# Quantumzhao/ParallelParsing

Hardware: AMD Instinct MI355X
Metric: FASTQ records/sec + decompressed MB/s, 50 GB .fastq.gz, 1/2/4/8 MI355X (higher is better)
Workload: dtype u8

## Files before the change

### parallelparsing_amd/csrc/ppg_inflate.hip

```cpp
#include <hip/hip_runtime.h>
#include <stdint.h>
#include <stdlib.h>
#include <stdio.h>
#include <type_traits>
#include "ppg_device.h"
#include "ppg_huffman.h"
#include <atomic>
#include <mutex>
#define PPG_SORT_SLOT 320

#define IX_RING_BYTES 65536u
#define IX_RING_MASK (IX_RING_BYTES - 1u)

template <int RB, int LBT, typename RingT = uint8_t>
struct __attribute__((aligned(16))) InflateLds {
    uint32_t stream[132];
    RingT ring[1u << RB];
    union {
        uint32_t lit[1 << LBT];
        uint32_t cl[1 << CB];
    };
    uint32_t dst[1 << DB];
    uint8_t lens[320];
    uint32_t cen[8];
    uint16_t dsort[32];
};

#ifdef PPG_IX_STATS
__device__ unsigned long long ppg_ixstat[16];
#endif

#ifdef PPG_STAMPS
__device__ unsigned long long ppg_stamp_acc[25];
#define PPG_STAMP(t) const uint64_t t = __builtin_amdgcn_s_memtime()
#else
#define PPG_STAMP(t)
#endif

__device__ __forceinline__ uint32_t rdlane(uint32_t v, uint32_t lane) {
    return (uint32_t)__builtin_amdgcn_readlane((int)v, (int)lane);
}

extern "C" __device__ int llvm_writelane(int, int, int) __asm("llvm.amdgcn.writelane");

__device__ __forceinline__ uint32_t bperm(uint32_t byte_addr, uint32_t v) {
    return (uint32_t)__builtin_amdgcn_ds_bpermute((int)byte_addr, (int)v);
}

struct Reader {
    const uint32_t *base;
    uint32_t nw;
    uint32_t sg;
    uint32_t wi;
    uint64_t bb;
    uint32_t bn;
};

__device__ __forceinline__ void lds_dma_dword(const uint32_t *src, const uint32_t *lds_base) {
    asm volatile("s_nop 0\n\tglobal_load_lds_dword %0, off" ::"v"(src), "{m0}"((uint32_t)(uintptr_t)lds_base)
                 : "memory");
}

__device__ __forceinline__ void st_issue(const Reader &r, uint32_t *stream, uint32_t g, int lane) {
    const uint32_t i = min(g * 32 + (uint32_t)lane, r.nw - 1);
    if (lane < 32) lds_dma_dword(r.base + i, stream + (g & 3) * 32);
    if ((g & 3) == 0 && lane < 4) lds_dma_dword(r.base + i, stream + 128);
}

__device__ __forceinline__ void st_enter(Reader &r, uint32_t *stream, uint32_t g, int lane) {
    if (g == r.sg || g + 1 == r.sg) return;
    if (g != r.sg + 1) {
        st_issue(r, stream, g, lane);
        st_issue(r, stream, g + 1, lane);
    }
    st_issue(r, stream, g + 2, lane);
    r.sg = g;
    asm volatile("s_waitcnt vmcnt(1)" ::: "memory");
}

__device__ __forceinline__ uint32_t rd_word(Reader &r, uint32_t *stream, uint32_t w, int lane) {
    st_enter(r, stream, w >> 5, lane);
    return uni(stream[w & 127]);
}

__device__ __forceinline__ void rd_seek(Reader &r, uint32_t *stream, uint32_t bit, int lane) {
    r.wi = bit >> 5;
    const uint32_t w = rd_word(r, stream, r.wi, lane);
    r.wi++;
    const uint32_t sh = bit & 31;
    r.bb = (uint64_t)(w >> sh);
    r.bn = 32 - sh;
}

__device__ __forceinline__ void rd_refill(Reader &r, uint32_t *stream, int lane) {
    if (r.bn <= 32) {
        const uint32_t w = rd_word(r, stream, r.wi, lane);
        r.wi++;
        r.bb |= (uint64_t)w << r.bn;
        r.bn += 32;
    }
}

__device__ __forceinline__ uint32_t rd_pos(const Reader &r) { return r.wi * 32 - r.bn; }

template <int RB>
__device__ __forceinline__ void flush_range(const uint8_t *ring, uint8_t *out, uint64_t glo, uint64_t ghi, int lane) {
    constexpr uint64_t RM = (1ull << RB) - 1;
    if (ghi <= glo) return;
    const uint64_t a = (glo + 15) & ~15ull, z = ghi & ~15ull;
    if (a >= z) {
        for (uint64_t g0 = glo; g0 < ghi; g0 += 64) {
            const uint64_t g = g0 + lane;
            if (g < ghi) out[g] = ring[g & RM];
        }
        return;
    }
    if (lane < (int)(a - glo)) out[glo + lane] = ring[(glo + lane) & RM];
    if (lane < (int)(ghi - z)) out[z + lane] = ring[(z + lane) & RM];
    for (uint64_t g0 = a; g0 < z; g0 += 1024) {
        const uint64_t g = g0 + (uint64_t)lane * 16;
        if (g < z) {
            uint4 v = *(const uint4 *)(ring + (g & RM));
            *(uint4 *)(out + g) = v;
        }
    }
}

template <int RB>
__device__ __forceinline__ void flush_range_sym(const uint16_t *ring, uint16_t *out, uint64_t glo, uint64_t ghi,
                                                int lane) {
    constexpr uint64_t RM = (1ull << RB) - 1;
    if (ghi <= glo) return;
    const uint64_t a = (glo + 7) & ~7ull, z = ghi & ~7ull;
    if (a >= z) {
        for (uint64_t g0 = glo; g0 < ghi; g0 += 64) {
            const uint64_t g = g0 + lane;
            if (g < ghi) out[g] = ring[g & RM];
        }
        return;
    }
    if (lane < (int)(a - glo)) out[glo + lane] = ring[(glo + lane) & RM];
    if (lane < (int)(ghi - z)) out[z + lane] = ring[(z + lane) & RM];
    for (uint64_t g0 = a; g0 < z; g0 += 512) {
        const uint64_t g = g0 + (uint64_t)lane * 8;
        if (g < z) *(uint4 *)(out + g) = *(const uint4 *)(ring + (g & RM));
    }
}

#define PPG_FILL 0x41414141u

__device__ __forceinline__ uint32_t zero_bytes(uint32_t x) {
    return ~(((x & 0x7F7F7F7Fu) + 0x7F7F7F7Fu) | x) & 0x80808080u;
}

__device__ __forceinline__ uint32_t nl_mask16(uint32_t w0, uint32_t w1, uint32_t w2, uint32_t w3) {
    const uint32_t n0 = zero_bytes(w0 ^ 0x0A0A0A0Au) >> 7, n1 = zero_bytes(w1 ^ 0x0A0A0A0Au) >> 7;
    const uint32_t n2 = zero_bytes(w2 ^ 0x0A0A0A0Au) >> 7, n3 = zero_bytes(w3 ^ 0x0A0A0A0Au) >> 7;
    const uint32_t lo = __builtin_amdgcn_udot4(n1, 0x80402010u, __builtin_amdgcn_udot4(n0, 0x08040201u, 0u, false), false);
    const uint32_t hi = __builtin_amdgcn_udot4(n3, 0x80402010u, __builtin_amdgcn_udot4(n2, 0x08040201u, 0u, false), false);
    return lo | (hi << 8);
}

__device__ __forceinline__ uint32_t wave_incl_scan(uint32_t x) {
    x += (uint32_t)__builtin_amdgcn_update_dpp(0, (int)x, 0x111, 0xF, 0xF, false);
    x += (uint32_t)__builtin_amdgcn_update_dpp(0, (int)x, 0x112, 0xF, 0xF, false);
    x += (uint32_t)__builtin_amdgcn_update_dpp(0, (int)x, 0x114, 0xF, 0xF, false);
    x += (uint32_t)__builtin_amdgcn_update_dpp(0, (int)x, 0x118, 0xF, 0xF, false);
    x += (uint32_t)__builtin_amdgcn_update_dpp(0, (int)x, 0x142, 0xA, 0xF, false);
    x += (uint32_t)__builtin_amdgcn_update_dpp(0, (int)x, 0x143, 0xC, 0xF, false);
    return x;
}

struct CensusOut {
    uint32_t *dst;
    uint32_t cap;
    uint32_t shift;
};

__device__ __forceinline__ void census_step(uint32_t *cen, const CensusOut &co, uint32_t w0, uint32_t w1, uint32_t w2,
                                            uint32_t w3, uint32_t p_lane, uint32_t lastbit, uint32_t nact, int lane) {
    const uint32_t m = nl_mask16(w0, w1, w2, w3);
    const uint32_t z = zero_bytes(w0) | zero_bytes(w1) | zero_bytes(w2) | zero_bytes(w3);
    const uint64_t L = __ballot((m >> lastbit) & 1u);
    const uint64_t F = __ballot(m & 1u);
    const uint64_t B = __ballot((m & (m << 1)) != 0u);
    const uint64_t Z = __ballot(z != 0u);
    uint32_t cnt = uni(cen[0]);
    const uint32_t prevnl = uni(cen[1]);
    uint32_t flags = uni(cen[2]);
    if (B | Z | (F & ((L << 1) | prevnl))) flags |= PPG_PF_SERIAL;
    if (Z) flags |= PPG_PF_NUL;
    const uint32_t c = (uint32_t)__builtin_popcount(m);
    const uint32_t incl = wave_incl_scan(c);
    const uint32_t total = rdlane(incl, 63);
    if (total) {
        uint32_t idx = cnt + incl - c;
        uint32_t mm = m;
        while (__ballot(mm != 0u)) {
            if (mm) {
                const uint32_t b = (uint32_t)__builtin_ctz(mm);
                mm &= mm - 1u;
                if (idx < co.cap) ((__attribute__((address_space(1))) uint32_t *)co.dst)[idx] = co.shift + p_lane + b;
                idx++;
            }
        }
        cnt += total;
        if (cnt > co.cap) flags |= PPG_PF_OVERFLOW;
    }
    if (lane == 0) {
        cen[0] = cnt;
        cen[1] = (uint32_t)(L >> (nact - 1)) & 1u;
        cen[2] = flags;
    }
}

__device__ __forceinline__ CensusOut census_out(const uint32_t *cen) {
    CensusOut co;
    co.cap = uni(cen[3]);
    co.shift = uni(cen[4]);
    co.dst = (uint32_t *)(((uint64_t)uni(cen[6]) << 32) | uni(cen[5]));
    return co;
}

template <int RB>
__device__ __forceinline__ void flush_census(const uint8_t *ring, uint8_t *out, uint64_t out_off, uint32_t lo,
                                             uint32_t hi, int lane, uint32_t *cen) {
    constexpr uint32_t RM = (1u << RB) - 1;
    const CensusOut co = census_out(cen);
    for (uint32_t p = lo; p < hi;) {
        const uint64_t g = out_off + p;
        const uint32_t left = hi - p;
        const uint32_t head = (uint32_t)(-g & 15);
        uint32_t w0 = PPG_FILL, w1 = PPG_FILL, w2 = PPG_FILL, w3 = PPG_FILL, lastbit, nact;
        if (head == 0 && left >= 16) {
            nact = min(left / 16, 64u);
            if ((uint32_t)lane < nact) {
                const uint4 v = *(const uint4 *)(ring + ((uint32_t)(g + 16 * lane) & RM));
                *(uint4 *)(out + g + 16 * lane) = v;
                w0 = v.x; w1 = v.y; w2 = v.z; w3 = v.w;
            }
            lastbit = 15;
            nact *= 16;
        } else {
            nact = min(head ? head : 64u, left);
            if ((uint32_t)lane < nact) {
                const uint8_t c = ring[(uint32_t)(g + lane) & RM];
                out[g + lane] = c;
                w0 = (PPG_FILL & ~255u) | c;
            }
            lastbit = 0;
        }
        census_step(cen, co, w0, w1, w2, w3, p + (lastbit ? 16 : 1) * (uint32_t)lane, lastbit,
                    lastbit ? nact / 16 : nact, lane);
        p += nact;
    }
}

template <bool IX = false, uint32_t IXM = IX_RING_MASK>
__device__ __forceinline__ uint32_t far_byte(const uint8_t *ob, uint32_t oa, const uint8_t *dict, int32_t p) {
    if constexpr (IX) {
        if (p >= 0) return ((const uint16_t *)ob)[(uint32_t)p & IXM];
        return 32768u + (uint32_t)p;
    } else {
        if (p >= 0) {
            const uint32_t q = oa + (uint32_t)p;
            return (*(const uint32_t *)(ob + (q & ~3u)) >> (8 * (q & 3))) & 255u;
        }
        return dict[32768u + (uint32_t)p];
    }
}

__device__ __forceinline__ uint32_t far_load(const uint8_t *base, uint32_t off) {
    uint32_t v;
    asm volatile("global_load_dword %0, %1, %2\n\ts_waitcnt vmcnt(0)" : "=&v"(v) : "v"(off), "s"(base) : "memory");
    return v;
}
__device__ __forceinline__ uint32_t far_load_u8(const uint8_t *base, uint32_t off) {
    uint32_t v;
    asm volatile("global_load_ubyte %0, %1, %2\n\ts_waitcnt vmcnt(0)" : "=&v"(v) : "v"(off), "s"(base) : "memory");
    return v;
}

template <int RB, bool IX, typename RingT, uint32_t IXM = IX_RING_MASK>
__device__ __forceinline__ void copy_match(RingT *ring, const uint8_t *ob, uint32_t oa, const uint8_t *dict,
                                           uint32_t rb0, uint32_t pos, uint32_t dist, uint32_t n, int lane) {
    constexpr uint32_t RM = (1u << RB) - 1;
    constexpr uint32_t REACH = (1u << RB) - 64;
    const uint32_t dst0 = rb0 + pos;
    if (dist + n <= REACH) {
        const uint32_t src0 = dst0 - dist;
        if (dist >= n) {
            for (uint32_t j0 = 0; j0 < n; j0 += 64) {
                const uint32_t j = j0 + lane;
                if (j < n) ring[(dst0 + j) & RM] = ring[(src0 + j) & RM];
            }
        } else {
            for (uint32_t j0 = 0; j0 < n; j0 += 64) {
                const uint32_t j = j0 + lane;
                if (j < n) ring[(dst0 + j) & RM] = ring[(src0 + j % dist) & RM];
            }
        }
    } else {
        for (uint32_t j0 = 0; j0 < n; j0 += 64) {
            const uint32_t j = j0 + lane;
            if (j < n) {
                const uint32_t back = dist - j;
                const int32_t rel = (int32_t)pos - (int32_t)back;
                uint32_t v;
                if (back + n <= REACH) v = ring[(dst0 - back) & RM];
                else v = far_byte<IX, IXM>(ob, oa, dict, rel);
                ring[(dst0 + j) & RM] = (RingT)v;
            }
        }
    }
}

template <int LBT>
__device__ __forceinline__ uint32_t spec_token(const uint32_t *lit, const uint32_t *dst, uint32_t lo, uint32_t hi,
                                               uint32_t lane) {
    const uint32_t e = lit[lo & ((1u << LBT) - 1)];
    const uint32_t e2 = e >> 8;
    const uint32_t xs = e2 - e;
    const uint32_t y = __builtin_amdgcn_alignbit(hi, lo, e2);
    uint32_t tke;
    asm("v_lshl_add_u32 %0, %1, 8, %2" : "=v"(tke) : "v"(__builtin_amdgcn_ubfe(lo, e, xs)), "v"(e2));
    const uint32_t d = dst[y & ((1u << DB) - 1)];
    const uint32_t dm1 = (d >> 16) + __builtin_amdgcn_ubfe(y, d, d >> 10);
    const uint32_t tlen = tke + ((d >> 5) & 31) + (dm1 << 17);
    const uint32_t lm = (uint32_t)((int32_t)(e << 25) >> 31);
    const uint32_t sd = (uint32_t)((int32_t)d >> 31);
    uint32_t t2, tok;
    asm("v_bfi_b32 %0, %1, %2, %3" : "=v"(t2) : "v"(sd), "v"(PPG_SPECIAL_TOKEN), "v"(tlen));
    asm("v_bfi_b32 %0, %1, %2, %3" : "=v"(tok) : "v"(lm), "v"(t2), "v"(e));
    return tok;
}
__device__ __forceinline__ void walk2_asm(uint32_t va, uint32_t vb, uint32_t &vtin, uint32_t &X, uint32_t &t,
                                          uint32_t &half) {
    uint32_t tmp;
    asm volatile(
        "1:\n\t"
        "v_readlane_b32 %[t], %[va], %[X]\n\t"
        "s_lshr_b32 m0, %[X], 8\n\t"
        "s_add_u32 %[X], %[t], %[X]\n\t"
        "s_and_b32 %[tmp], %[X], 0x1c0c0\n\t"
        "v_writelane_b32 %[vtin], %[t], m0\n\t"
        "s_cbranch_scc1 4f\n\t"
        "v_readlane_b32 %[t], %[va], %[X]\n\t"
        "s_lshr_b32 m0, %[X], 8\n\t"
        "s_add_u32 %[X], %[t], %[X]\n\t"
        "s_and_b32 %[tmp], %[X], 0x1c0c0\n\t"
        "v_writelane_b32 %[vtin], %[t], m0\n\t"
        "s_cbranch_scc0 1b\n"
        "4:\n\t"
        "s_mov_b32 %[h], 0\n\t"
        "s_and_b32 %[tmp], %[X], 0x1c080\n\t"
        "s_cbranch_scc1 3f\n\t"
        "s_sub_u32 %[X], %[X], 64\n\t"
        "s_mov_b32 %[h], 64\n"
        "2:\n\t"
        "v_readlane_b32 %[t], %[vb], %[X]\n\t"
        "s_lshr_b32 m0, %[X], 8\n\t"
        "s_add_u32 %[X], %[t], %[X]\n\t"
        "s_and_b32 %[tmp], %[X], 0x1c0c0\n\t"
        "v_writelane_b32 %[vtin], %[t], m0\n\t"
        "s_cbranch_scc1 3f\n\t"
        "v_readlane_b32 %[t], %[vb], %[X]\n\t"
        "s_lshr_b32 m0, %[X], 8\n\t"
        "s_add_u32 %[X], %[t], %[X]\n\t"
        "s_and_b32 %[tmp], %[X], 0x1c0c0\n\t"
        "v_writelane_b32 %[vtin], %[t], m0\n\t"
        "s_cbranch_scc0 2b\n"
        "3:"
        : [vtin] "+v"(vtin), [X] "+s"(X), [t] "=&s"(t), [tmp] "=&s"(tmp), [h] "=&s"(half)
        : [va] "v"(va), [vb] "v"(vb)
        : "m0", "scc");
}
__device__ __forceinline__ uint32_t latch_limit(uint32_t x, uint32_t lim) {
    uint32_t r;
    asm("s_bitcmp1_b32 %1, 7\n\ts_cselect_b32 %0, 0, %2" : "=s"(r) : "s"(uni(x)), "s"(uni(lim)) : "scc");
    return r;
}


template <int RB, int LBT, bool IX, bool CEN, bool IXF = false>
__global__ __launch_bounds__(64) __attribute__((amdgpu_num_sgpr(80), amdgpu_waves_per_eu(8, 8))) void ppg_inflate_kernel(const uint32_t *__restrict__ comp, uint64_t nwords,
                                                         const PpgInflateJob *__restrict__ jobs,
                                                         const uint8_t *__restrict__ dicts, uint8_t *__restrict__ out,
                                                         PpgInflateResult *__restrict__ res, int njobs,
                                                         PpgBlockEnd *__restrict__ blk, uint32_t *__restrict__ nls,
                                                         uint16_t *__restrict__ gsort) {
    constexpr uint32_t RING = 1u << RB;
    constexpr uint32_t RM = RING - 1;
    constexpr uint32_t UNIT = RB >= 13 ? 4096u : RING / 2;
    static_assert(RB >= 10 && RB <= 15, "ring of 1..32 KiB");
    using RingT = typename std::conditional<IX, uint16_t, uint8_t>::type;
    constexpr uint32_t IXM = IXF ? 0xFFFFFFFFu : IX_RING_MASK;
    static_assert(!IXF || IX, "IXF is a pass-1 (IX) form");
    __shared__ InflateLds<RB, LBT, RingT> S;
    const int lane = threadIdx.x;
    const int k = blockIdx.x;
    if (k >= njobs) return;
    uint16_t *const lit_sorted = gsort + (size_t)k * PPG_SORT_SLOT;
    uint16_t *const dst_sorted = S.dsort;
    uint16_t *const lit_tmp = (uint16_t *)S.dst, *const cl_tmp = (uint16_t *)S.dst, *const dst_tmp = (uint16_t *)S.lens;
#ifdef PPG_STAMPS
    const uint64_t tk0 = __builtin_amdgcn_s_memtime();
    uint64_t sx_spec = 0, sx_nspec = 0, sx_flush = 0, sx_nflush = 0, sx_hdr = 0, sx_nhdr = 0, sx_hp = 0, sx_nhp = 0;
#endif
    const PpgInflateJob J = jobs[k];
    const uint64_t out_off = J.out_off;
    const uint32_t len = IX ? 0xFFFFFFFFu : (uint32_t)J.out_len;
    const uint32_t ixcap = IXF ? (uint32_t)J.out_len : 0xF0000000u;
    const uint32_t rb0 = (uint32_t)out_off;
    const uint8_t *dict = dicts + J.dict_off;
    const uint8_t *ob = IX ? out + 2 * out_off : out + (out_off & ~3ull);
    const uint32_t oa = IX ? 0u : (uint32_t)(out_off & 3);

    if constexpr (IX) {
        for (uint32_t w0 = 0; w0 < RING; w0 += 64) {
            const uint32_t w = w0 + lane;
            S.ring[(rb0 - RING + w) & RM] = (uint16_t)(32768u - RING + w);
        }
    } else {
        for (uint32_t w0 = 0; w0 < RING / 4; w0 += 64) {
            const uint32_t w = w0 + lane;
            const uint32_t v = *(const uint32_t *)(dict + 32768 - RING + 4 * w);
            const uint32_t slot = rb0 - RING + 4 * w;
#pragma unroll
            for (int q = 0; q < 4; q++) S.ring[(slot + q) & RM] = (uint8_t)(v >> (8 * q));
        }
    }
    constexpr bool census = CEN && !IX;
    if (census && lane == 0) {
        const uint64_t d = (uint64_t)(uintptr_t)(nls + J.nl_off);
        S.cen[0] = 0;
        S.cen[1] = J.prev_byte == '\n';
        S.cen[2] = 0;
        S.cen[3] = J.nl_cap;
        S.cen[4] = J.raw_shift;
        S.cen[5] = (uint32_t)d;
        S.cen[6] = (uint32_t)(d >> 32);
    }
    __syncthreads();

    const uint64_t w0abs = (J.bit_start >> 5) & ~127ull;
    Reader r;
    r.sg = 0x7FFFFFF0u;
    r.base = comp + w0abs;
    r.nw = (uint32_t)min(nwords > w0abs ? nwords - w0abs : 1ull, 0xFFFFFFFFull);
    const uint32_t bit_limit = (uint32_t)min(J.bit_limit - w0abs * 32, 0xFFFFFFFFull);
    rd_seek(r, S.stream, (uint32_t)(J.bit_start - w0abs * 32), lane);

    const uint64_t lanes_le = lane == 63 ? ~0ull : ((2ull << lane) - 1ull);

    uint32_t pos = 0;
    uint32_t fl_done = 0;
    uint32_t fl_next = UNIT - (uint32_t)(out_off % UNIT);
    int status = ST_OK, flags = 0, last = 0, in_block = 0;
    Canon clit = {0, 0, 0}, cdst = {0, 0, 0};
#ifdef PPG_IX_STATS
    uint64_t ix_unk = 0;
    uint32_t ix_last = 0;
#endif
    auto flush = [&](uint32_t lo, uint32_t hi) {
        if constexpr (IX) {
#ifdef PPG_IX_STATS
            for (uint32_t p0 = lo; p0 < hi; p0 += 64) {
                const uint32_t p = p0 + (uint32_t)lane;
                const uint64_t b = __ballot(p < hi && S.ring[(rb0 + p) & RM] < 0x8000u);
                ix_unk += (uint64_t)__popcll(b);
                if (b) ix_last = p0 + 64u - (uint32_t)__clzll(b);
            }
#endif
            const uint64_t g = out_off + (lo & IXM);
            flush_range_sym<RB>(S.ring, (uint16_t *)out, g, g + (hi - lo), lane);
        } else {
            if constexpr (census) {
                flush_census<RB>(S.ring, out, out_off, lo, hi, lane, S.cen);
            } else {
                flush_range<RB>(S.ring, out, out_off + lo, out_off + hi, lane);
            }
        }
    };
    uint32_t nblk = 0;
#ifdef PPG_STAMPS
    uint64_t sa_dec = 0, sa_walk = 0, sa_rd = 0, sa_far = 0, sa_dep = 0, sa_tail = 0, sa_rounds = 0, sa_farr = 0;
    uint64_t hs_dec = 0, hs_walk = 0, hs_look = 0, hs_fin = 0, hs_words = 0, hs_emit = 0, hs_rounds = 0;
#endif
#ifdef PPG_STATS
    uint32_t st_rounds = 0, st_tokens = 0, st_spec = 0, st_short = 0, st_far = 0, st_dep = 0, st_dbl = 0,
             st_blit = 0, st_beob = 0, st_bmatch = 0;
#endif
    auto block_end = [&](uint32_t e) -> bool {
        if (nblk >= J.blk_cap) { flags |= PPG_FLAG_BLK_FULL; return false; }
        if (lane == 0) blk[J.blk_off + nblk] = PpgBlockEnd{w0abs * 32 + e, pos};
        nblk++;
        return w0abs * 32 + e < J.stop_bit;
    };


    while (pos < len && !last) {
        r.sg = uni(r.sg);
        r.wi = uni(r.wi);
        r.bb = uni64(r.bb);
        r.bn = uni(r.bn);
        pos = uni(pos);
        fl_done = uni(fl_done);
        fl_next = uni(fl_next);
        status = (int)uni((uint32_t)status);
#ifdef PPG_STAMPS
        const uint64_t th0 = __builtin_amdgcn_s_memtime();
#endif
        rd_refill(r, S.stream, lane);
        last = (int)br_take(r, 1);
        const uint32_t type = br_take(r, 2);
        if (type == 0) {
            br_take(r, r.bn & 7);
            rd_refill(r, S.stream, lane);
            const uint32_t slen = br_take(r, 16), nlen = br_take(r, 16);
            if ((slen ^ 0xFFFFu) != nlen) { status = ST_DATA_ERROR; break; }
            const uint32_t bytepos = rd_pos(r) >> 3;
            const uint8_t *c8 = (const uint8_t *)r.base + bytepos;
            const uint32_t remain = min(slen, len - pos);
            if ((uint64_t)bytepos + remain > (uint64_t)r.nw * 4) { status = ST_DATA_ERROR; break; }
            uint32_t copied = 0;
            while (copied < remain) {
                const uint32_t piece = min(remain - copied, (uint32_t)UNIT);
                for (uint32_t j0 = 0; j0 < piece; j0 += 64) {
                    const uint32_t j = j0 + lane;
                    if (j < piece) S.ring[(rb0 + pos + j) & RM] = (RingT)((IX ? 0x8000u : 0u) | c8[copied + j]);
                }
                pos += piece;
                copied += piece;
                if (pos >= fl_next) {
                    flush(fl_done, fl_next);
                    fl_done = fl_next;
                    fl_next += UNIT;
                }
            }
            rd_seek(r, S.stream, (bytepos + copied) * 8, lane);
            if (copied < slen) break;
            in_block = 0;
            if constexpr (IX) {
                if (!block_end((bytepos + copied) * 8)) break;
            }
            continue;
        }
        if (type == 3) { status = ST_DATA_ERROR; break; }
        if (type == 1) {
            for (int s0 = 0; s0 < 320; s0 += 64) {
                const int s = s0 + lane;
                uint8_t L;
                if (s < 144) L = 8; else if (s < 256) L = 9; else if (s < 280) L = 7; else if (s < 288) L = 8;
                else L = 5;
                S.lens[s] = L;
            }
            __syncthreads();
            build_table<LBT>(S.lens, 288, S.lit, &clit, lit_tmp, TAB_LIT, lane, lit_sorted);
            build_table<DB>(S.lens + 288, 32, S.dst, &cdst, dst_tmp, TAB_DST, lane, dst_sorted);
        } else {
            asm volatile("s_setprio 2");
            rd_refill(r, S.stream, lane);
            const uint32_t hlit = br_take(r, 5) + 257, hdist = br_take(r, 5) + 1, hclen = br_take(r, 4) + 4;
            if (hlit > 286 || hdist > 30) { status = ST_DATA_ERROR; break; }
            if (lane < 19) S.lens[lane] = 0;
            __syncthreads();
            for (uint32_t i = 0; i < hclen; i++) {
                rd_refill(r, S.stream, lane);
                const uint32_t v = br_take(r, 3);
                if (lane == 0) S.lens[c_clorder[i]] = (uint8_t)v;
            }
            __syncthreads();
            if (build_table<CB>(S.lens, 19, S.cl, nullptr, cl_tmp, TAB_CL, lane) != 0) { status = ST_DATA_ERROR; break; }
            uint32_t idx = 0;
            const uint32_t total = hlit + hdist;
            bool bad = false;
            while (idx < total) {
                rd_refill(r, S.stream, lane);
                const uint32_t e = uni(S.cl[(uint32_t)r.bb & ((1u << CB) - 1)]);
                const uint32_t L = e & 15;
                if (L == 0) { bad = true; break; }
                br_take(r, L);
                const uint32_t sym = e >> 8;
                uint32_t val = 0, rep = 1;
                if (sym < 16) { val = sym; }
                else if (sym == 16) {
                    if (idx == 0) { bad = true; break; }
                    val = uni(S.lens[idx - 1]);
                    rep = 3 + br_take(r, 2);
                } else if (sym == 17) { rep = 3 + br_take(r, 3); }
                else { rep = 11 + br_take(r, 7); }
                if (idx + rep > total) { bad = true; break; }
                for (uint32_t j0 = 0; j0 < rep; j0 += 64)
                    if (j0 + lane < rep) S.lens[idx + j0 + lane] = (uint8_t)val;
                idx += rep;
            }
            __syncthreads();
            if (bad) { status = ST_DATA_ERROR; break; }
            if (uni(S.lens[256]) == 0) { status = ST_DATA_ERROR; break; }
            if (build_table<LBT>(S.lens, (int)hlit, S.lit, &clit, lit_tmp, TAB_LIT, lane, lit_sorted) != 0) { status = ST_DATA_ERROR; break; }
            if (build_table<DB>(S.lens + hlit, (int)hdist, S.dst, &cdst, dst_tmp, TAB_DST, lane, dst_sorted) != 0) { status = ST_DATA_ERROR; break; }
        }
        in_block = 1;
#ifdef PPG_STAMPS
        sx_hdr += __builtin_amdgcn_s_memtime() + 0 * (uint64_t)__builtin_amdgcn_readfirstlane(S.lit[lane]) - th0;
        sx_nhdr++;
#endif
        asm volatile("s_setprio 0");
        r.sg = uni(r.sg);
        r.wi = uni(r.wi);
        r.bb = uni64(r.bb);
        r.bn = uni(r.bn);
        pos = uni(pos);
        fl_done = uni(fl_done);
        fl_next = uni(fl_next);

        uint32_t bp = rd_pos(r);
#ifdef PPG_STAMPS
        uint64_t st_w0 = 0;
#endif
        uint32_t cn = 0, cw = 0;

        struct Round { uint32_t vtin, off, adv, tl, xr; };
        struct Words { uint32_t x0, x1, x2, x3, x4; };
        auto words = [&](uint32_t bp) -> Words {
            const uint32_t *sw = S.stream + __builtin_amdgcn_ubfe(bp + (uint32_t)lane, 5u, 7u);
            return Words{sw[0], sw[1], sw[2], sw[3], sw[4]};
        };
        auto decode = [&](auto hot, uint32_t bp, uint32_t cn, uint32_t cw, uint32_t pos, const Words &W) -> Round {
            constexpr bool HOT = decltype(hot)::value;
            uint32_t s = 0, off = cn, t = 0, half = 0;
            uint32_t tl = cw, xr = 0;
            uint32_t vtin = (uint32_t)llvm_writelane((int)cw, 0, 0);
            if (__builtin_expect(off < (HOT ? 64u : min(64u, len - pos)), 1)) {
                const uint32_t o = bp + (uint32_t)lane;
                const uint32_t x0 = W.x0, x1 = W.x1, x2 = W.x2, x3 = W.x3, x4 = W.x4;
                const uint32_t vta = spec_token<LBT>(S.lit, S.dst, __builtin_amdgcn_alignbit(x1, x0, o),
                                                     __builtin_amdgcn_alignbit(x2, x1, o), (uint32_t)lane);
                const uint32_t vtb = spec_token<LBT>(S.lit, S.dst, __builtin_amdgcn_alignbit(x3, x2, o),
                                                     __builtin_amdgcn_alignbit(x4, x3, o), (uint32_t)lane);

                constexpr uint32_t STOP = 0x1C0C0u;
                uint32_t X;
#ifdef PPG_STAMPS
                st_w0 = __builtin_amdgcn_s_memtime() + 0 * (uint64_t)__builtin_amdgcn_readfirstlane(vta ^ vtb);
#endif
                if (HOT || len - pos >= 64) {
                    X = off << 8;
                    asm volatile("s_setprio 2");
                    walk2_asm(vta, vtb, vtin, X, tl, half);
                    if constexpr (!HOT) asm volatile("s_setprio 1");
                    off = (X >> 8) & 511u;
                } else {
                    const uint32_t cl = 64u - (len - pos);
                    X = (off + cl) << 8;
                    do {
                        t = rdlane(vta, X);
                        vtin = (uint32_t)llvm_writelane((int)t, (int)((X >> 8) - cl), (int)vtin);
                        X += t;
                    } while ((X & STOP) == 0u);
                    if ((X & (STOP & ~0x40u)) == 0u) {
                        X -= 64;
                        half = 64;
                        do {
                            t = rdlane(vtb, X);
                            vtin = (uint32_t)llvm_writelane((int)t, (int)((X >> 8) - cl), (int)vtin);
                            X += t;
                        } while ((X & STOP) == 0u);
                    }
                    off = ((X >> 8) & 511u) - cl;
                    tl = t;
                }
                xr = X;
                s = half + (X & 127u);
            }
            return Round{vtin, off, s, tl, xr};
        };

        st_enter(r, S.stream, bp >> 10, lane);
        Words W = words(bp);
        auto one_round = [&]() -> uint32_t {
            constexpr bool HOT = false;
            PPG_STAMP(t0);
            const Round R = decode(std::false_type{}, bp, cn, cw, pos, W);
            st_enter(r, S.stream, (bp + R.adv) >> 10, lane);
            W = words(bp + R.adv);
#ifdef PPG_STAMPS
            const uint64_t t1 = __builtin_amdgcn_s_memtime() + 0 * (uint64_t)__builtin_amdgcn_readfirstlane(R.vtin);
            if (st_w0 < t0) st_w0 = t1;
            sa_dec += st_w0 - t0;
            sa_walk += t1 - st_w0;
            sa_rounds++;
#endif
#ifdef PPG_STATS
            st_rounds++;
            st_tokens += (uint32_t)__popcll(__ballot(R.vtin != 0));
            if (R.xr & 128u) st_spec++;
            if (R.off < 64) st_short++;
#endif
            const uint32_t tot = HOT ? R.off : min(R.off, len - pos);
            const uint32_t rout = min(tot, 64u);
            const uint64_t mo = __ballot(R.vtin != 0);
            {
                uint32_t sj4;
                asm("v_mad_i32_i24 %0, %1, -4, %2" : "=v"(sj4) : "v"((uint32_t)__builtin_clzll(mo & lanes_le)), "s"(252u));
                const uint32_t inf = bperm(sj4, R.vtin);
                const int32_t jj = lane - 1 - (int32_t)(inf >> 17);
                const uint32_t rv = S.ring[(rb0 + pos + (uint32_t)jj) & RM];
                uint32_t val;
                if constexpr (IX) val = ((inf >> 8) & 511u) != 1u ? rv : (0x8000u | ((inf >> 17) & 255u));
                else val = ((inf >> 8) & 511u) != 1u ? rv : ((inf >> 17) & 255u);
                const bool far = jj < -(int32_t)(RING - 64);
                const uint64_t fm = __ballot(far);
#ifdef PPG_STATS
                if (fm) st_far++;
#endif
#ifdef PPG_STAMPS
                const uint64_t t2 = __builtin_amdgcn_s_memtime() + 0 * (uint64_t)__builtin_amdgcn_readfirstlane(val);
                sa_rd += t2 - t1;
#endif
                if (fm) {
                  {
                    const int32_t p = (int32_t)pos + jj;
                    const bool fo = far && p >= 0;
                    if constexpr (IX) {
                        const uint32_t q = 2u * ((uint32_t)p & IXM);
                        const uint32_t w = far_load(ob, fo ? (q & ~3u) : 0u);
                        val = fo ? __builtin_amdgcn_ubfe(w, q << 3, 16u) : val;
                    } else {
                        const uint32_t b = far_load_u8(ob, fo ? (uint32_t)jj + (pos + oa) : 0u);
                        val = fo ? b : val;
                    }
                    const bool fd = far && p < 0;
                    const uint64_t dm = fm & __ballot(p < 0);
                    if (dm) {
                        uint32_t db;
                        if constexpr (IX) db = 32768u + (uint32_t)p;
                        else db = dict[fd ? 32768u + (uint32_t)p : 0u];
                        val = fd ? db : val;
                    }
                  }
                }
#ifdef PPG_STAMPS
                const uint64_t t3 = __builtin_amdgcn_s_memtime() + 0 * (uint64_t)__builtin_amdgcn_readfirstlane(val);
                sa_far += t3 - t2;
                sa_farr += fm ? 1 : 0;
#endif
                const bool dep = jj >= 0;
                if (__ballot(dep)) {
                    int32_t ptr = dep ? jj : lane;
#ifdef PPG_STATS
                    st_dep++;
#endif
                    for (;;) {
#ifdef PPG_STATS
                        st_dbl++;
#endif
                        const int32_t p2 = (int32_t)bperm((uint32_t)ptr << 2, (uint32_t)ptr);
                        if (!__ballot(p2 != ptr)) break;
                        ptr = p2;
                    }
                    val = bperm((uint32_t)ptr << 2, val);
                }
                S.ring[(rb0 + pos + lane) & RM] = (RingT)val;
#ifdef PPG_STAMPS
                const uint64_t t4 = __builtin_amdgcn_s_memtime() + 0 * (uint64_t)__builtin_amdgcn_readfirstlane(val);
                sa_dep += t4 - t3;
                st_w0 = t4;
#endif
            }
            cn = tot - rout;
            cw = R.tl & ~(511u << 8);
            pos += rout;
            bp += R.adv;
            asm volatile("s_setprio 0");
            if constexpr (IX) {
                if (bp > bit_limit || pos > ixcap) { status = ST_DATA_ERROR; return 128u; }
            }
#ifdef PPG_STAMPS
            sa_tail += __builtin_amdgcn_s_memtime() + 0 * (uint64_t)bp - st_w0;
            st_w0 = 0;
#endif
            return R.xr;
        };
        auto hot_pipe = [&](auto early, uint32_t limh) -> uint32_t {
            constexpr bool EARLY = decltype(early)::value;
            uint32_t p_val = 0, p_b = 0, p_pos = pos, lim_r;
            int32_t p_jj = -1;
            auto finish = [&]() {
                uint32_t val = p_val;
                if constexpr (IX) {
                    const uint32_t q = 2u * ((p_pos + (uint32_t)p_jj) & IXM);
                    uint32_t fv = __builtin_amdgcn_ubfe(p_b, q << 3, 16u);
                    if constexpr (EARLY) {
                        const int32_t p = (int32_t)p_pos + p_jj;
                        fv = p < 0 ? 32768u + (uint32_t)p : fv;
                    }
                    val = p_jj < -(int32_t)(RING - 64) ? fv : val;
                } else {
                    val = p_jj < -(int32_t)(RING - 64) ? p_b : val;
                }
                const bool dep = p_jj >= 0;
                if (__ballot(dep)) {
                    int32_t ptr = dep ? p_jj : lane;
                    for (;;) {
                        const int32_t p2 = (int32_t)bperm((uint32_t)ptr << 2, (uint32_t)ptr);
                        if (!__ballot(p2 != ptr)) break;
                        ptr = p2;
                    }
                    val = bperm((uint32_t)ptr << 2, val);
                }
                S.ring[(rb0 + p_pos + lane) & RM] = (RingT)val;
            };
            do {
                PPG_STAMP(h0);
                const Round R = decode(std::true_type{}, bp, cn, cw, pos, W);
#ifdef PPG_STAMPS
                const uint64_t h1 = __builtin_amdgcn_s_memtime() + 0 * (uint64_t)__builtin_amdgcn_readfirstlane(R.vtin);
                if (st_w0 < h0) st_w0 = h1;
                hs_dec += st_w0 - h0;
                hs_walk += h1 - st_w0;
                hs_rounds++;
#endif
                const uint32_t rout = min(R.off, 64u);
                const uint64_t mo = __ballot(R.vtin != 0);
                uint32_t sj4;
                asm("v_mad_i32_i24 %0, %1, -4, %2" : "=v"(sj4) : "v"((uint32_t)__builtin_clzll(mo & lanes_le)), "s"(252u));
                const uint32_t inf = bperm(sj4, R.vtin);
                asm volatile("s_setprio 0");
#ifdef PPG_STAMPS
                const uint64_t h2 = __builtin_amdgcn_s_memtime() + 0 * (uint64_t)__builtin_amdgcn_readfirstlane(inf);
                hs_look += h2 - h1;
#endif
                finish();
                if constexpr (!EARLY && !IX) {
                    if (pos >= fl_next) {
                        flush(fl_done, fl_next);
                        fl_done = fl_next;
                        fl_next += UNIT;
                    }
                }
#ifdef PPG_STAMPS
                const uint64_t h3 = __builtin_amdgcn_s_memtime() + 0 * (uint64_t)__builtin_amdgcn_readfirstlane(
                                                                       S.ring[(rb0 + p_pos + lane) & RM]);
                hs_fin += h3 - h2;
#endif
                st_enter(r, S.stream, (bp + R.adv) >> 10, lane);
                W = words(bp + R.adv);
#ifdef PPG_STAMPS
                const uint64_t h4 = __builtin_amdgcn_s_memtime() + 0 * (uint64_t)__builtin_amdgcn_readfirstlane(W.x4);
                hs_words += h4 - h3;
#endif
                const int32_t jj = lane - 1 - (int32_t)(inf >> 17);
                const uint32_t rv = S.ring[(rb0 + pos + (uint32_t)jj) & RM];
                if constexpr (IX) p_val = ((inf >> 8) & 511u) != 1u ? rv : (0x8000u | ((inf >> 17) & 255u));
                else p_val = ((inf >> 8) & 511u) != 1u ? rv : ((inf >> 17) & 255u);
                const bool far = jj < -(int32_t)(RING - 64);
                if constexpr (IX) {
                    const uint32_t q = 2u * ((pos + (uint32_t)jj) & IXM);
                    const bool ld = EARLY ? far && (int32_t)pos + jj >= 0 : far;
                    p_b = *(const uint32_t *)(ob + (uint64_t)(ld ? (q & ~3u) : 0u));
                } else if constexpr (EARLY) {
                    const int32_t p = (int32_t)pos + jj;
                    const uint8_t *src = p >= 0 ? ob + (oa + (uint32_t)p) : dict + (uint32_t)(32768 + p);
                    p_b = *(far ? src : ob);
                } else {
                    p_b = ob[(uint64_t)(far ? (uint32_t)jj + (pos + oa) : 0u)];
                }
                p_jj = jj;
                p_pos = pos;
                cn = R.off - rout;
                cw = R.tl & ~(511u << 8);
                pos += rout;
                bp += R.adv;
                asm volatile("s_setprio 0");
                lim_r = latch_limit(R.xr, limh);
                if constexpr (IX) {
                    if (bp > bit_limit || pos > ixcap) { status = ST_DATA_ERROR; lim_r = 0; }
                }
#ifdef PPG_STAMPS
                hs_emit += __builtin_amdgcn_s_memtime() + 0 * (uint64_t)__builtin_amdgcn_readfirstlane(p_b + lim_r) - h4;
                st_w0 = 0;
#endif
            } while (pos < lim_r);
            finish();
            return lim_r;
        };
        for (;;) {
            bool spec_ = false;
            const uint32_t lim = min(len, fl_next);
            uint32_t lim_r;
            {
                const uint32_t limh = min(fl_next, len > 322u ? len - 322u : 0u);
                if (pos < 32768u && pos < limh) {
                    const uint32_t lime = min(limh, 32768u);
#ifdef PPG_STAMPS
                    const uint64_t tq0 = __builtin_amdgcn_s_memtime();
#endif
                    lim_r = hot_pipe(std::true_type{}, lime);
#ifdef PPG_STAMPS
                    sx_hp += __builtin_amdgcn_s_memtime() + 0 * (uint64_t)lim_r - tq0;
                    sx_nhp++;
#endif
                    spec_ = lim_r == 0u;
                }
                const uint32_t limp = IX ? limh : (len > 322u ? len - 322u : 0u);
                if (!spec_ && pos >= 32768u && pos < limp) {
#ifdef PPG_STAMPS
                    const uint64_t tq0 = __builtin_amdgcn_s_memtime();
#endif
                    lim_r = hot_pipe(std::false_type{}, limp);
#ifdef PPG_STAMPS
                    sx_hp += __builtin_amdgcn_s_memtime() + 0 * (uint64_t)lim_r - tq0;
                    sx_nhp++;
#endif
                    spec_ = lim_r == 0u;
                }
                if (!spec_ && pos < lim) {
                    do {
                        lim_r = latch_limit(one_round(), lim);
                    } while (pos < lim_r);
                    spec_ = lim_r == 0u;
                }
            }
            if constexpr (IX) {
                if (status != ST_OK) break;
            }
            if (pos >= fl_next) {
#ifdef PPG_STAMPS
                const uint64_t tf0 = __builtin_amdgcn_s_memtime();
#endif
                flush(fl_done, fl_next);
                fl_done = fl_next;
                fl_next += UNIT;
#ifdef PPG_STAMPS
                sx_flush += __builtin_amdgcn_s_memtime() + 0 * (uint64_t)__builtin_amdgcn_readfirstlane(S.cen[0]) - tf0;
                sx_nflush++;
#endif
            }
            if (!spec_) {
                if (pos < len) continue;
                break;
            }
#ifdef PPG_STAMPS
            const uint64_t ts0 = __builtin_amdgcn_s_memtime();
            sx_nspec++;
#endif
            asm volatile("s_setprio 2");
            rd_seek(r, S.stream, bp, lane);
            rd_refill(r, S.stream, lane);
            int sym;
            uint32_t ml = 0;
            {
                const uint32_t e = uni(S.lit[(uint32_t)r.bb & ((1u << LBT) - 1)]);
                if (!(e & 0x80u)) {
                    const uint32_t L = e & 15u;
                    br_take(r, L);
                    if (e & 0x40u) {
                        ml = ((e >> 16) & 0x1FFu) + br_take(r, ((e >> 8) & 0xFFu) - L);
                        sym = 257;
                    } else {
                        sym = (int)((e >> 17) & 0xFFu);
                    }
                } else {
                    sym = canon_decode(r, clit, lit_sorted, lane);
                    if (sym > 256 && sym < 286) {
                        ml = c_lbase[sym - 257] + br_take(r, c_lext[sym - 257]);
                        sym = 257;
                    }
                }
            }
#ifdef PPG_STATS
            if (sym < 256) st_blit++; else if (sym == 256) st_beob++; else st_bmatch++;
#endif
            if (sym < 0 || sym > 257) { status = ST_DATA_ERROR; break; }
            if (sym < 256) {
                if (lane == 0) S.ring[(rb0 + pos) & RM] = (RingT)((IX ? 0x8000u : 0u) | (uint32_t)sym);
                pos++;
            } else if (sym == 256) {
                in_block = 0;
                bp = rd_pos(r);
                break;
            } else {
                rd_refill(r, S.stream, lane);
                uint32_t ds;
                const uint32_t d = uni(S.dst[(uint32_t)r.bb & ((1u << DB) - 1)]);
                if (d != ~0u) {
                    br_take(r, d & 15u);
                    ds = (d >> 16) + 1u + br_take(r, (d >> 10) & 31u);
                } else {
                    const int dsym = canon_decode(r, cdst, dst_sorted, lane);
                    if (dsym < 0 || dsym >= 30) { status = ST_DATA_ERROR; break; }
                    ds = c_dbase[dsym] + br_take(r, c_dext[dsym]);
                }
                const uint32_t n = min(ml, len - pos);
                copy_match<RB, IX, RingT, IXM>(S.ring, ob, oa, dict, rb0, pos, ds, n, lane);
                pos += n;
            }
            bp = rd_pos(r);
            if (pos >= fl_next) {
                flush(fl_done, fl_next);
                fl_done = fl_next;
                fl_next += UNIT;
            }
            st_enter(r, S.stream, bp >> 10, lane);
            W = words(bp);
            asm volatile("s_setprio 0");
#ifdef PPG_STAMPS
            sx_spec += __builtin_amdgcn_s_memtime() + 0 * (uint64_t)__builtin_amdgcn_readfirstlane(W.x4) - ts0;
#endif
            if (pos >= len) break;
        }
        if (status != ST_OK) break;
        rd_seek(r, S.stream, bp, lane);
        if constexpr (IX) {
            if (in_block) { status = ST_DATA_ERROR; break; }
            if (!block_end(bp)) break;
        }
    }
    flush(fl_done, pos);

    uint32_t end_bit = rd_pos(r);
    if (end_bit > bit_limit) {
        flags |= PPG_FLAG_OVERRUN;
        if (status == ST_OK) status = ST_DATA_ERROR;
    }
    if (!IX && status == ST_OK && in_block && pos == len) {
        rd_refill(r, S.stream, lane);
        if (canon_decode(r, clit, lit_sorted, lane) == 256) end_bit = rd_pos(r);
        else flags |= PPG_FLAG_NO_EOB;
    }
#ifdef PPG_STATS
    if (!IX && lane == 0 && k < 4)
        printf("PPG_STATS chunk %d: bytes %u rounds %u tokens %u spec %u short %u far %u dep %u dbl %u "
               "bitserial lit %u eob %u match %u\n", k, pos, st_rounds, st_tokens, st_spec, st_short, st_far, st_dep,
               st_dbl, st_blit, st_beob, st_bmatch);
#endif
#ifdef PPG_IX_STATS
    if (IX && lane == 0) {
        atomicAdd(&ppg_ixstat[0], (unsigned long long)ix_unk);
        atomicAdd(&ppg_ixstat[1], (unsigned long long)ix_last);
        atomicAdd(&ppg_ixstat[2], (unsigned long long)pos);
        atomicAdd(&ppg_ixstat[3], 1ull);
        atomicAdd(&ppg_ixstat[4 + min(9u, (uint32_t)(10ull * ix_last / max(pos, 1u)))], 1ull);
        atomicMax(&ppg_ixstat[14], (unsigned long long)ix_last);
    }
#endif
#ifdef PPG_STAMPS
    if (!IX && lane == 0) {
        atomicAdd(&ppg_stamp_acc[0], (unsigned long long)sa_dec);
        atomicAdd(&ppg_stamp_acc[1], (unsigned long long)sa_walk);
        atomicAdd(&ppg_stamp_acc[2], (unsigned long long)sa_rd);
        atomicAdd(&ppg_stamp_acc[3], (unsigned long long)sa_far);
        atomicAdd(&ppg_stamp_acc[4], (unsigned long long)sa_dep);
        atomicAdd(&ppg_stamp_acc[5], (unsigned long long)sa_tail);
        atomicAdd(&ppg_stamp_acc[6], (unsigned long long)sa_rounds);
        atomicAdd(&ppg_stamp_acc[7], (unsigned long long)sa_farr);
        atomicAdd(&ppg_stamp_acc[8], (unsigned long long)hs_dec);
        atomicAdd(&ppg_stamp_acc[9], (unsigned long long)hs_walk);
        atomicAdd(&ppg_stamp_acc[10], (unsigned long long)hs_look);
        atomicAdd(&ppg_stamp_acc[11], (unsigned long long)hs_fin);
        atomicAdd(&ppg_stamp_acc[12], (unsigned long long)hs_words);
        atomicAdd(&ppg_stamp_acc[13], (unsigned long long)hs_emit);
        atomicAdd(&ppg_stamp_acc[14], (unsigned long long)hs_rounds);
        atomicAdd(&ppg_stamp_acc[15], (unsigned long long)(__builtin_amdgcn_s_memtime() - tk0));
        atomicAdd(&ppg_stamp_acc[16], (unsigned long long)sx_spec);
        atomicAdd(&ppg_stamp_acc[17], (unsigned long long)sx_nspec);
        atomicAdd(&ppg_stamp_acc[18], (unsigned long long)sx_flush);
        atomicAdd(&ppg_stamp_acc[19], (unsigned long long)sx_nflush);
        atomicAdd(&ppg_stamp_acc[20], (unsigned long long)sx_hdr);
        atomicAdd(&ppg_stamp_acc[21], (unsigned long long)sx_nhdr);
        atomicAdd(&ppg_stamp_acc[22], 1ull);
        atomicAdd(&ppg_stamp_acc[23], (unsigned long long)sx_hp);
        atomicAdd(&ppg_stamp_acc[24], (unsigned long long)sx_nhp);
    }
#endif
    if (lane == 0) {
        res[k].produced = pos;
        res[k].end_bit = w0abs * 32 + end_bit;
        res[k].status = status;
        res[k].flags = flags;
        res[k].nblocks = nblk;
        res[k].last = (uint32_t)last;
        res[k].newlines = census ? S.cen[0] : 0;
        res[k].pflags = census ? S.cen[2] : 0;
    }
}

static hipError_t gsort_alloc(hipStream_t s, int njobs, uint16_t **p) {
    static std::mutex mu;
    static hipMemPool_t pools[64] = {};
    static bool tried[64] = {};
    int dev = 0;
    hipError_t e = hipGetDevice(&dev);
    if (e != hipSuccess) return e;
    const size_t bytes = (size_t)njobs * PPG_SORT_SLOT * sizeof(uint16_t);
    hipMemPool_t pool = nullptr;
    if (dev >= 0 && dev < 64) {
        std::lock_guard<std::mutex> lk(mu);
        if (!tried[dev]) {
            tried[dev] = true;
            hipMemPoolProps props = {};
            props.allocType = hipMemAllocationTypePinned;
            props.handleTypes = hipMemHandleTypeNone;
            props.location.type = hipMemLocationTypeDevice;
            props.location.id = dev;
            if (hipMemPoolCreate(&pools[dev], &props) == hipSuccess) {
                uint64_t t = ~0ull;
                (void)hipMemPoolSetAttribute(pools[dev], hipMemPoolAttrReleaseThreshold, &t);
            } else {
                pools[dev] = nullptr;
                (void)hipGetLastError();
            }
        }
        pool = pools[dev];
    }
    if (pool) return hipMallocFromPoolAsync((void **)p, bytes, pool, s);
    return hipMallocAsync((void **)p, bytes, s);
}
#define PPG_GSORT_BEGIN(s, njobs)                          \
    uint16_t *gsort = nullptr;                             \
    {                                                      \
        const hipError_t ge = gsort_alloc(s, njobs, &gsort); \
        if (ge != hipSuccess) return ge;                   \
    }
#define PPG_GSORT_END(s) (void)hipFreeAsync(gsort, s)

#define PPG_VARIANTS(X) X(10, 8) X(10, 9) X(11, 9) X(11, 8) X(12, 9) X(12, 8) X(13, 9) X(15, 9)

#ifdef PPG_STAMPS
struct PpgStampPrinter;
static void ppg_stamp_dump(hipStream_t s);
#define PPG_STAMP_DUMP(s) ppg_stamp_dump(s)
#else
#define PPG_STAMP_DUMP(s)
#endif

size_t ppg_inflate_lds_bytes(int ring_bits, int lit_bits) {
#define X(R, L) if (ring_bits == R && lit_bits == L) return sizeof(InflateLds<R, L>);
    PPG_VARIANTS(X)
#undef X
    return 0;
}

hipError_t ppg_launch_inflate(hipStream_t s, int ring_bits, int lit_bits, const uint32_t *comp, uint64_t nwords,
                              const PpgInflateJob *jobs, const uint8_t *dicts, uint8_t *out, PpgInflateResult *res,
                              int njobs, uint32_t *nls) {
    if (njobs <= 0) return hipSuccess;
    static const bool no_census = getenv("PPG_PROBE_NO_CENSUS") != nullptr;
    if (no_census) nls = nullptr;
#define X(R, L)                                                                                               \
    if (ring_bits == R && lit_bits == L) {                                                                    \
        PPG_GSORT_BEGIN(s, njobs);                                                                            \
        if (nls)                                                                                              \
            hipLaunchKernelGGL((ppg_inflate_kernel<R, L, false, true>), dim3(njobs), dim3(64),                \
                               0, s, comp, nwords, jobs, dicts, out, res, njobs, nullptr, nls, gsort);          \
        else                                                                                                  \
            hipLaunchKernelGGL((ppg_inflate_kernel<R, L, false, false>), dim3(njobs), dim3(64),               \
                               0, s, comp, nwords, jobs, dicts, out, res, njobs, nullptr, nls, gsort);          \
        const hipError_t le = hipGetLastError();                                                              \
        PPG_GSORT_END(s);                                                                                     \
        PPG_STAMP_DUMP(s);                                                                                    \
        return le;                                                                                            \
    }
    PPG_VARIANTS(X)
#undef X
    return hipErrorInvalidValue;
}

#ifdef PPG_STAMPS
struct PpgStampPrinter {
    static void dump(hipStream_t s) {
        unsigned long long h[25] = {0};
        if (hipStreamSynchronize(s) != hipSuccess) return;
        if (hipMemcpyFromSymbol(h, HIP_SYMBOL(ppg_stamp_acc), sizeof h) != hipSuccess) return;
        const unsigned long long z[25] = {0};
        (void)hipMemcpyToSymbol(HIP_SYMBOL(ppg_stamp_acc), z, sizeof z);
        const double r = h[6] ? (double)h[6] : 1.0;
        fprintf(stderr, "PPG_STAMPS rounds %llu far-rounds %llu cycles/round: decode %.1f walk %.1f read %.1f far %.1f "
                        "dep+write %.1f tail %.1f total %.1f\n", h[6], h[7], h[0] / r, h[1] / r, h[2] / r, h[3] / r,
                h[4] / r, h[5] / r, (h[0] + h[1] + h[2] + h[3] + h[4] + h[5]) / r);
        const double q = h[14] ? (double)h[14] : 1.0;
        fprintf(stderr, "PPG_STAMPS hot rounds %llu cycles/round: decode %.1f walk %.1f lookup %.1f finish %.1f "
                        "words %.1f emit+tail %.1f total %.1f\n", h[14], h[8] / q, h[9] / q, h[10] / q, h[11] / q,
                h[12] / q, h[13] / q, (h[8] + h[9] + h[10] + h[11] + h[12] + h[13]) / q);
        const double T = h[15] ? (double)h[15] : 1.0;
        const double hot = h[8] + h[9] + h[10] + h[11] + h[12] + h[13], gen = h[0] + h[1] + h[2] + h[3] + h[4] + h[5];
        fprintf(stderr, "PPG_STAMPS jobs %llu wave cycles %.4g: hot rounds %.1f%% general rounds %.1f%% bit-serial tokens "
                        "%.1f%% (%llu, %.0f cycles each) flushes %.1f%% (%llu, %.0f each) block headers %.1f%% (%llu, %.0f "
                        "each) other %.1f%%\n", h[22], T, 100 * hot / T, 100 * gen / T, 100 * h[16] / T, h[17],
                h[16] / (h[17] ? (double)h[17] : 1.0), 100 * h[18] / T, h[19], h[18] / (h[19] ? (double)h[19] : 1.0),
                100 * h[20] / T, h[21], h[20] / (h[21] ? (double)h[21] : 1.0),
                100 * (T - hot - gen - h[16] - h[18] - h[20]) / T);
        fprintf(stderr, "PPG_STAMPS pipelined-loop calls %llu: %.1f%% of wave cycles inside them, %.0f cycles per call "
                        "outside their rounds (entry, the pending round's finish, exit)\n", h[24], 100 * h[23] / T,
                (h[23] - hot) / (h[24] ? (double)h[24] : 1.0));
    }
};
#endif

hipError_t ppg_launch_inflate_ix(hipStream_t s, const uint32_t *comp, uint64_t nwords, const PpgInflateJob *jobs,
                                 const uint8_t *dicts, uint8_t *out, PpgInflateResult *res, PpgBlockEnd *blk,
                                 int njobs) {
    if (njobs <= 0) return hipSuccess;
    PPG_GSORT_BEGIN(s, njobs);
    hipLaunchKernelGGL((ppg_inflate_kernel<10, 8, true, false>), dim3(njobs), dim3(64), 0, s, comp,
                       nwords, jobs, dicts, out, res, njobs, blk, nullptr, gsort);
    const hipError_t le = hipGetLastError();
    PPG_GSORT_END(s);
    if (le != hipSuccess) return le;
#ifdef PPG_IX_STATS
    {
        unsigned long long h[16] = {0};
        if (hipStreamSynchronize(s) == hipSuccess && hipMemcpyFromSymbol(h, HIP_SYMBOL(ppg_ixstat), sizeof h) == hipSuccess) {
            const unsigned long long z[16] = {0};
            (void)hipMemcpyToSymbol(HIP_SYMBOL(ppg_ixstat), z, sizeof z);
            fprintf(stderr, "PPG_IX_STATS jobs %llu bytes %llu unknown %llu (%.4f%%) mean last %.0f max last %llu tenths", h[3],
                    h[2], h[0], 100.0 * h[0] / (h[2] ? h[2] : 1), (double)h[1] / (h[3] ? h[3] : 1), h[14]);
            for (int i = 4; i < 14; i++) fprintf(stderr, " %llu", h[i]);
            fprintf(stderr, "\n");
        }
    }
#endif
    return hipGetLastError();
}

#ifdef PPG_STAMPS
static void ppg_stamp_dump(hipStream_t s) { PpgStampPrinter::dump(s); }
#endif

hipError_t ppg_launch_inflate_ixf(hipStream_t s, const uint32_t *comp, uint64_t nwords, const PpgInflateJob *jobs,
                                  const uint8_t *dicts, uint8_t *out, PpgInflateResult *res, PpgBlockEnd *blk,
                                  int njobs) {
    if (njobs <= 0) return hipSuccess;
    PPG_GSORT_BEGIN(s, njobs);
    hipLaunchKernelGGL((ppg_inflate_kernel<10, 8, true, false, true>), dim3(njobs), dim3(64), 0, s, comp, nwords, jobs,
                       dicts, out, res, njobs, blk, nullptr, gsort);
    const hipError_t le = hipGetLastError();
    PPG_GSORT_END(s);
    return le;
}

template <int RB>
__global__ __launch_bounds__(64) void ppg_materialize_kernel(const uint16_t *__restrict__ sym,
                                                             const uint8_t *__restrict__ wins,
                                                             const PpgMatInfo *__restrict__ mi,
                                                             const PpgInflateJob *__restrict__ jobs,
                                                             uint8_t *__restrict__ out, PpgInflateResult *__restrict__ res,
                                                             int njobs, uint32_t *__restrict__ nls) {
    constexpr uint32_t RING = 1u << RB, RM = RING - 1, UNIT = RING / 2, PER = UNIT / 64;
    __shared__ __attribute__((aligned(16))) uint8_t W[32768];
    __shared__ __attribute__((aligned(16))) uint8_t ring[RING];
    __shared__ uint32_t cen[8];
    const int k = blockIdx.x, lane = threadIdx.x;
    if (k >= njobs) return;
    const PpgInflateJob J = jobs[k];
    const PpgMatInfo M = mi[k];
    for (uint32_t i = 16u * (uint32_t)lane; i < 32768u; i += 1024u)
        *(uint4 *)&W[i] = *(const uint4 *)(wins + M.win_off + i);
    if (lane == 0) {
        const uint64_t d = (uint64_t)(uintptr_t)(nls + J.nl_off);
        cen[0] = 0;
        cen[2] = 0;
        cen[3] = J.nl_cap;
        cen[4] = J.raw_shift;
        cen[5] = (uint32_t)d;
        cen[6] = (uint32_t)(d >> 32);
    }
    __syncthreads();
    if (lane == 0) cen[1] = (M.prev > 255u ? W[32767] : M.prev) == '\n';
    const uint32_t len = (uint32_t)J.out_len;
    const uint64_t out_off = J.out_off;
    const uint16_t *sy = sym + M.sym_off;
    auto unit_end = [&](uint32_t p) { return min(len, p + (UNIT - (uint32_t)((out_off + p) & (UNIT - 1)))); };
    uint32_t v[PER];
    auto fetch = [&](uint32_t p0, uint32_t p1) {
#pragma unroll
        for (uint32_t i = 0; i < PER; i++) {
            const uint32_t p = p0 + (uint32_t)lane + 64u * i;
            v[i] = p < p1 ? (uint32_t)sy[p] : 0x8000u;
        }
    };
    uint32_t p0 = 0, p1 = unit_end(0);
    fetch(p0, p1);
    while (p0 < len) {
#pragma unroll
        for (uint32_t i = 0; i < PER; i++) {
            const uint32_t p = p0 + (uint32_t)lane + 64u * i;
            if (p < p1) ring[(uint32_t)(out_off + p) & RM] = (uint8_t)((v[i] & 0x8000u) ? v[i] : W[v[i] & 32767u]);
        }
        __syncthreads();
        const uint32_t q1 = unit_end(p1);
        fetch(p1, q1);
        flush_census<RB>(ring, out, out_off, p0, p1, lane, cen);
        __syncthreads();
        p0 = p1;
        p1 = q1;
    }
    if (lane == 0) {
        res[k].produced = len;
        res[k].end_bit = M.end_bit;
        res[k].status = 0;
        res[k].flags = 0;
        res[k].nblocks = M.nblocks;
        res[k].last = M.last;
        res[k].newlines = cen[0];
        res[k].pflags = cen[2];
    }
}

hipError_t ppg_launch_materialize(hipStream_t s, const uint16_t *sym, const uint8_t *wins, const PpgMatInfo *mi,
                                  const PpgInflateJob *jobs, uint8_t *out, PpgInflateResult *res, int njobs,
                                  uint32_t *nls) {
    if (njobs <= 0) return hipSuccess;
    hipLaunchKernelGGL(ppg_materialize_kernel<12>, dim3(njobs), dim3(64), 0, s, sym, wins, mi, jobs, out, res, njobs, nls);
    return hipGetLastError();
}
```

Measured before the change: 1.026 billion.

## Decode long-code tokens in-round to keep hot pipeline running

Adds a scalar long_token decoder, used when the wave-parallel decode round stops because it hits a token whose code is too long for the fast table. It decodes that single literal or match token, including the canonical-decode fallback, then resumes the hot pipe loop instead of leaving it for the slow bitserial path. The goal is to avoid the costly pipeline exit and re-entry on rare long codes, at the price of more code in the hot loop and extra register pressure. A stats counter tracks how often this path is taken.

```diff
diff --git a/parallelparsing_amd/csrc/ppg_inflate.hip b/parallelparsing_amd/csrc/ppg_inflate.hip
--- a/parallelparsing_amd/csrc/ppg_inflate.hip
+++ b/parallelparsing_amd/csrc/ppg_inflate.hip
@@ -489,7 +489,7 @@
 #endif
 #ifdef PPG_STATS
     uint32_t st_rounds = 0, st_tokens = 0, st_spec = 0, st_short = 0, st_far = 0, st_dep = 0, st_dbl = 0,
-             st_blit = 0, st_beob = 0, st_bmatch = 0;
+             st_blit = 0, st_beob = 0, st_bmatch = 0, st_inround = 0;
 #endif
     auto block_end = [&](uint32_t e) -> bool {
         if (nblk >= J.blk_cap) { flags |= PPG_FLAG_BLK_FULL; return false; }
@@ -783,6 +783,43 @@
 #endif
             return R.xr;
         };
+        auto long_token = [&](uint32_t lo, uint32_t hi) -> uint32_t {
+            struct { uint64_t bb; uint32_t bn; } q = {((uint64_t)hi << 32) | lo, 64u};
+            int sym;
+            uint32_t ml = 0;
+            const uint32_t e = uni(S.lit[lo & ((1u << LBT) - 1)]);
+            if (!(e & 0x80u)) {
+                const uint32_t L = e & 15u;
+                br_take(q, L);
+                if (e & 0x40u) {
+                    ml = ((e >> 16) & 0x1FFu) + br_take(q, ((e >> 8) & 0xFFu) - L);
+                    sym = 257;
+                } else {
+                    sym = (int)((e >> 17) & 0xFFu);
+                }
+            } else {
+                sym = canon_decode(q, clit, lit_sorted, lane);
+                if (sym > 256 && sym < 286) {
+                    const uint32_t i = (uint32_t)sym - 257u, x = i < 8u || i == 28u ? 0u : (i - 4u) >> 2;
+                    ml = (i < 8u ? 3u + i : i == 28u ? 258u : 3u + ((4u + (i & 3u)) << x)) + br_take(q, x);
+                    sym = 257;
+                }
+            }
+            if (sym < 0 || sym == 256 || sym > 257) return 0u;
+            if (sym < 256) return (64u - q.bn) | (1u << 8) | ((0x100u | (uint32_t)sym) << 17);
+            uint32_t dm1;
+            const uint32_t d = uni(S.dst[(uint32_t)q.bb & ((1u << DB) - 1)]);
+            if (d != ~0u) {
+                br_take(q, d & 15u);
+                dm1 = (d >> 16) + br_take(q, (d >> 10) & 31u);
+            } else {
+                const int dsym = canon_decode(q, cdst, dst_sorted, lane);
+                if (dsym < 0 || dsym >= 30) return 0u;
+                const uint32_t j = (uint32_t)dsym, x = j < 4u ? 0u : (j - 2u) >> 1;
+                dm1 = (j < 4u ? j : (2u + (j & 1u)) << x) + br_take(q, x);
+            }
+            return (64u - q.bn) | (ml << 8) | (dm1 << 17);
+        };
         auto hot_pipe = [&](auto early, uint32_t limh) -> uint32_t {
             constexpr bool EARLY = decltype(early)::value;
             uint32_t p_val = 0, p_b = 0, p_pos = pos, lim_r;
@@ -812,6 +849,26 @@
                 }
                 S.ring[(rb0 + p_pos + lane) & RM] = (RingT)val;
             };
+            auto carry_long = [&]() -> bool {
+                if constexpr (IX) return false;
+                if (lim_r != 0u) return false;
+                asm volatile("s_setprio 2");
+                const uint32_t tw = long_token(uni(__builtin_amdgcn_alignbit(W.x1, W.x0, bp)),
+                                               uni(__builtin_amdgcn_alignbit(W.x2, W.x1, bp)));
+                if (tw) {
+#ifdef PPG_STATS
+                    st_inround++;
+#endif
+                    cn = (tw >> 8) & 511u;
+                    cw = cn == 1u ? tw : tw & ~(511u << 8);
+                    bp += tw & 255u;
+                    st_enter(r, S.stream, bp >> 10, lane);
+                    W = words(bp);
+                    lim_r = limh;
+                }
+                asm volatile("s_setprio 0");
+                return pos < lim_r;
+            };
             do {
                 PPG_STAMP(h0);
                 const Round R = decode(std::true_type{}, bp, cn, cw, pos, W);
@@ -882,7 +939,7 @@
                 hs_emit += __builtin_amdgcn_s_memtime() + 0 * (uint64_t)__builtin_amdgcn_readfirstlane(p_b + lim_r) - h4;
                 st_w0 = 0;
 #endif
-            } while (pos < lim_r);
+            } while (pos < lim_r || carry_long());
             finish();
             return lim_r;
         };
@@ -1033,8 +1090,8 @@
 #ifdef PPG_STATS
     if (!IX && lane == 0 && k < 4)
         printf("PPG_STATS chunk %d: bytes %u rounds %u tokens %u spec %u short %u far %u dep %u dbl %u "
-               "bitserial lit %u eob %u match %u\n", k, pos, st_rounds, st_tokens, st_spec, st_short, st_far, st_dep,
-               st_dbl, st_blit, st_beob, st_bmatch);
+               "bitserial lit %u eob %u match %u in-round long codes %u\n", k, pos, st_rounds, st_tokens, st_spec,
+               st_short, st_far, st_dep, st_dbl, st_blit, st_beob, st_bmatch, st_inround);
 #endif
 #ifdef PPG_IX_STATS
     if (IX && lane == 0) {
```

Measured after the change: 1.036 billion, median of 6. No clear change (+1.0%).
